# wazzuck/multimodal-image-transformer

Measured on AMD Instinct MI355X. Metric: image-caption pairs/sec (train step), 6L/d512 decoder + ViT-B/16, 1/2/4/8 GPU, higher is better.
Workload: dtype bf16; 1 GPU; configs[1]: 6L d512 decoder + ViT-B/16 (197 patches), batch 64/GPU, seq_len 64; global_batch=64, seq_len=64, vocab=10000, memory_mode=patches, parallelism=dp1

## Files before the change

### include/mit_hip.h

```cpp
#ifndef MIT_HIP_H
#define MIT_HIP_H

#include <stdint.h>

#ifdef __cplusplus
extern "C" {
#endif

#define MIT_OK 0
#define MIT_ERR_INVALID 1
#define MIT_ERR_HIP 2

enum { MIT_F32 = 0, MIT_BF16 = 1 };
enum { MIT_K_CONTIG = 0, MIT_MN_CONTIG = 1 };
enum { MIT_ACT_NONE = 0, MIT_ACT_RELU = 1, MIT_ACT_GELU = 2, MIT_ACT_QUICK_GELU = 3 };
#define MIT_ARGMAX_SLOTS 16
enum { MIT_DECODE_ATTN_BH = 0, MIT_DECODE_ATTN_ROWS = 1, MIT_DECODE_ATTN_ROWS_NT = 2 };

const char* mit_last_error(void);
int mit_abi_version(void);

void* mit_plan_begin(void);
void* mit_plan_end(void);
long mit_plan_size(const void* plan);
// ... 79 lines not shown
  long k_row, k_batch;
  const void* v;
  long v_row, v_batch;
  void* o;
  long o_row, o_batch;
  float* lse;
  const int64_t* key_tokens;
  long tok_batch;
  int pad_idx;
  int causal;
  float scale;
  float drop_p;
  const uint64_t* seed;
  uint32_t site;
} mit_attn_args;
int mit_attention_fwd(int dtype, long B, long H, long Lq, long Lk, long Dh, const mit_attn_args* a, void* stream);

typedef struct {
  const void* dout;
  long do_row, do_batch;
  void* dq;
  long dq_row, dq_batch;
  void* dk;
  long dk_row, dk_batch;
  void* dv;
  long dv_row, dv_batch;
  float* delta_ws;
} mit_attn_grads;
int mit_attention_bwd(int dtype, long B, long H, long Lq, long Lk, long Dh, const mit_attn_args* a,
                      const mit_attn_grads* g, void* stream);

int mit_attention_set_index_limit(double limit);

enum { MIT_ATTN_GENERIC = 0, MIT_ATTN_FWD_MFMA = 1, MIT_ATTN_FWD_HEAD = 2, MIT_ATTN_FWD_HEAD_DROP = 3 };
enum { MIT_ATTN_BWD_MFMA = 1, MIT_ATTN_BWD_HEAD = 2 };
typedef struct {
  int fwd, fwd_nw, fwd_lkp;
  int bwd, bwd_nw, bwd_lkp;
} mit_attn_plan;
int mit_attention_plan(int dtype, long B, long H, long Lq, long Lk, long Dh, const mit_attn_args* a,
                       const mit_attn_grads* g, mit_attn_plan* plan);

int mit_im2col(int dtype, long B, long C, long H, long W, long P, const float* img, void* out, long kpad, void* stream);
int mit_vit_assemble(int dtype, long B, long np, long E, const void* patch, const float* cls, const float* pos, void* h,
                     void* stream);
enum { MIT_ELT_SCALAR = 0, MIT_ELT_VEC8 = 1 };
int mit_im2col_plan(int dtype, long B, long C, long H, long W, long P, const float* img, const void* out, long kpad);
int mit_vit_assemble_plan(int dtype, long B, long np, long E, const void* patch, const float* cls, const float* pos,
                          const void* h);

int mit_embed_fwd(int dtype, long B, long T, long d, const int64_t* tokens, const void* table, float scale,
                  const float* pe, float drop_p, const uint64_t* seed, uint32_t site, void* out, void* stream);
long mit_embed_plan_ints(long n);
int mit_embed_plan(const int64_t* tokens, long n, int* plan, void* stream);
int mit_embed_plan_keys_per_thread(long n);
int mit_embed_bwd(int dtype, long B, long T, long d, const int64_t* tokens, const void* dx, float scale, float drop_p,
                  const uint64_t* seed, uint32_t site, int pad_idx, const int* plan, float* dtable, void* stream);

enum { MIT_CE_BLOCK = 0, MIT_CE_ROWS = 1 };
int mit_cross_entropy_plan(int dtype, long rows, long V, const void* logits, long ld, const float* row_loss);
int mit_count_targets(const int64_t* targets, long n, int ignore_index, float* count, void* stream);
int mit_cross_entropy(int dtype, long rows, long V, void* logits, long ld, const int64_t* targets, int ignore_index,
                      const float* count, float* loss_sum, int want_grad, float* row_loss, void* stream);
int mit_scalar_div(const float* a, const float* b, float* out, void* stream);

int mit_colsum(int dtype, long M, long N, const void* dy, long ld, float* out, int accumulate, float* ws, void* stream);
long mit_colsum_ws_floats(long M, long N);
// ... 157 lines not shown
```

### multimodal-image-transformer_amd/csrc/attention.hip

```cpp
#include "common.h"

namespace {

constexpr int D = 64;

struct AttnK {
  const void* q;
  long q_row, q_batch;
  const void* k;
  long k_row, k_batch;
  const void* v;
  long v_row, v_batch;
  void* o;
  long o_row, o_batch;
  float* lse;
  const int64_t* tok;
  long tok_batch;
  int pad;
  int causal;
  float scale;
  const uint64_t* seed;
  uint32_t site;
  uint32_t thresh;
  float dscale;
// ... 387 lines not shown
#pragma unroll
  for (int i = 0; i < 4; ++i) {
    typedef __attribute__((ext_vector_type(4))) __bf16 bf16x4;
    bf16x4 o4 = {(bf16)(ot[i][0] * inv), (bf16)(ot[i][1] * inv), (bf16)(ot[i][2] * inv), (bf16)(ot[i][3] * inv)};
    *(bf16x4*)(O + i * 16 + g * 4) = o4;
  }
  if (a.lse && g == 0) a.lse[(b * H + h) * Lq + qi] = (m + __log2f(l)) * 0.6931471805599453f;
}

constexpr int HK_MAX = 640;
constexpr int HS = 4;
constexpr int HS_DROP = 8;

__device__ __forceinline__ float xmax_rows(float v) {
  const auto a = __builtin_amdgcn_permlane16_swap(__float_as_uint(v), __float_as_uint(v), false, false);
  v = __builtin_fmaxf(__uint_as_float(a[0]), __uint_as_float(a[1]));
  const auto b = __builtin_amdgcn_permlane32_swap(__float_as_uint(v), __float_as_uint(v), false, false);
  return __builtin_fmaxf(__uint_as_float(b[0]), __uint_as_float(b[1]));
}
__device__ __forceinline__ float xsum_rows(float v) {
  const auto a = __builtin_amdgcn_permlane16_swap(__float_as_uint(v), __float_as_uint(v), false, false);
  v = __uint_as_float(a[0]) + __uint_as_float(a[1]);
  const auto b = __builtin_amdgcn_permlane32_swap(__float_as_uint(v), __float_as_uint(v), false, false);
  return __uint_as_float(b[0]) + __uint_as_float(b[1]);
}
__device__ __forceinline__ float max16(const float (&s)[16]) {
  const float a = __builtin_fmaxf(__builtin_fmaxf(s[0], s[1]), s[2]), b = __builtin_fmaxf(__builtin_fmaxf(s[3], s[4]), s[5]);
  const float c = __builtin_fmaxf(__builtin_fmaxf(s[6], s[7]), s[8]), d = __builtin_fmaxf(__builtin_fmaxf(s[9], s[10]), s[11]);
  const float e = __builtin_fmaxf(__builtin_fmaxf(s[12], s[13]), s[14]);
  return __builtin_fmaxf(__builtin_fmaxf(__builtin_fmaxf(a, b), c), __builtin_fmaxf(__builtin_fmaxf(d, e), s[15]));
}
constexpr bf16x8 ones8 = {(bf16)1.0f, (bf16)1.0f, (bf16)1.0f, (bf16)1.0f, (bf16)1.0f, (bf16)1.0f, (bf16)1.0f, (bf16)1.0f};

template <bool DROP>
__global__ __attribute__((amdgpu_flat_work_group_size(64, DROP ? 512 : 1024))) void attn_fwd_head(long H, long Lq, long Lk, AttnK a, int kbytes, int vbytes,
                                                      int lkp) {
  extern __shared__ __attribute__((aligned(16))) char lds[];
  char* Ks = lds;
  char* Vs = lds + (long)lkp * 128;
  constexpr int HSN = DROP ? HS_DROP : HS;
  const int tid = threadIdx.x, lane = tid & 63, w = tid >> 6, g = lane >> 4, nw = blockDim.x >> 6;
  const long h = blockIdx.x, b = blockIdx.y;
  MIT_DASSERT(h < H && Lk <= lkp && lkp <= HK_MAX && Lq > 0);
  const bf16* Kb = (const bf16*)a.k + b * a.k_batch + h * D;
  const bf16* Vb = (const bf16*)a.v + b * a.v_batch + h * D;
  const __amdgpu_buffer_rsrc_t rk = __builtin_amdgcn_make_buffer_rsrc((void*)Kb, (short)0, kbytes, 0x00020000);
  const __amdgpu_buffer_rsrc_t rv = __builtin_amdgcn_make_buffer_rsrc((void*)Vb, (short)0, vbytes, 0x00020000);
  const int nid = lkp * 8;
  for (int base = tid; base < nid; base += HSN * (int)blockDim.x) {
    u32x4 kv[HSN], vv[HSN];
#pragma unroll
    for (int u = 0; u < HSN; ++u) {
      const int id = base + u * (int)blockDim.x, r = id >> 3, c = id & 7;
      const bool ok = r < Lk;
      kv[u] = __builtin_bit_cast(u32x4, __builtin_amdgcn_raw_buffer_load_b128(
                                            rk, (int)(ok ? (uint32_t)((r * a.k_row + c * 8) * 2) : A_OOB), 0, 0));
      vv[u] = __builtin_bit_cast(u32x4, __builtin_amdgcn_raw_buffer_load_b128(
                                            rv, (int)(ok ? (uint32_t)((r * a.v_row + c * 8) * 2) : A_OOB), 0, 0));
    }
#pragma unroll
    for (int u = 0; u < HSN; ++u) {
      const int id = base + u * (int)blockDim.x, r = id >> 3, c = id & 7;
      if (id < nid) {
        *(u32x4*)(Ks + koff_k(r, c)) = kv[u];
        *(u32x4*)(Vs + koff_v(r, c * 16)) = vv[u];
      }
    }
  }
  __syncthreads();

  const float sl2 = a.scale * 1.4426950408889634f;
  const uint64_t key = DROP ? site_key(a.seed, a.site) : 0ull;
  const int nqt = (int)((Lq + 15) / 16);
  const int q = (lane & 15) >> 2, pp = lane & 3;
  const int kofs = koff_k(lane & 15, g);
  const int kofs1 = koff_k(lane & 15, 4 + g);
  int vofs[4][2];
#pragma unroll
  for (int i = 0; i < 4; ++i) {
    const int colb = (i * 16 + 4 * pp) * 2;
    vofs[i][0] = koff_v(g * 4 + q, colb);
    vofs[i][1] = koff_v(16 + g * 4 + q, colb);
  }
  for (int qt = w; qt < nqt; qt += nw) {
    const long qi = (long)qt * 16 + (lane & 15);
    const bool qlive = qi < Lq;
    bf16x8 qf[2];
    {
      const bf16* Qr = (const bf16*)a.q + b * a.q_batch + h * D + (qlive ? qi : 0) * a.q_row;
#pragma unroll
      for (int kk = 0; kk < 2; ++kk) {
        u32x4 v = *(const u32x4*)(Qr + kk * 32 + g * 8);
        if (!qlive) v = u32x4{0u, 0u, 0u, 0u};
        qf[kk] = __builtin_bit_cast(bf16x8, v);
      }
    }
    const uint32_t rowbase = ((uint32_t)(b * H + h) * (uint32_t)Lq + (uint32_t)qi) * (uint32_t)Lk + (uint32_t)(g * 4);
    const uint32_t kf = key_fold(key);
    f32x4 ot[4];
#pragma unroll
    for (int i = 0; i < 4; ++i) ot[i] = f32x4{0.f, 0.f, 0.f, 0.f};
    float m = -INFINITY, l = 0.f;
    f32x4 lacc = {0.f, 0.f, 0.f, 0.f};
    const char* Kc = Ks;
    const char* Vc = Vs;
    int j0 = 0;
    const int ilk = (int)Lk;
    for (; j0 + 64 <= lkp; j0 += 64, Kc += 64 * 128, Vc += 64 * 128) {
      f32x4 st[4];
#pragma unroll
      for (int nb = 0; nb < 4; ++nb) {
        const u32x4 k0 = *(const u32x4*)(Kc + nb * 2048 + kofs);
        const u32x4 k1 = *(const u32x4*)(Kc + nb * 2048 + kofs1);
        st[nb] = __builtin_amdgcn_mfma_f32_16x16x32_bf16(__builtin_bit_cast(bf16x8, k0), qf[0],
                                                          f32x4{0.f, 0.f, 0.f, 0.f}, 0, 0, 0);
        st[nb] = __builtin_amdgcn_mfma_f32_16x16x32_bf16(__builtin_bit_cast(bf16x8, k1), qf[1], st[nb], 0, 0, 0);
      }
      s16x8 vv[2][4];
#pragma unroll
      for (int hh = 0; hh < 2; ++hh)
#pragma unroll
        for (int i = 0; i < 4; ++i) {
          s16x4 lo = __builtin_amdgcn_ds_read_tr16_b64_v4i16(LDS_PTR(s16x4, Vc + hh * 4096 + vofs[i][0]));
          s16x4 hi = __builtin_amdgcn_ds_read_tr16_b64_v4i16(LDS_PTR(s16x4, Vc + hh * 4096 + vofs[i][1]));
          vv[hh][i] = s16x8{lo[0], lo[1], lo[2], lo[3], hi[0], hi[1], hi[2], hi[3]};
        }
      float s[16];
#pragma unroll
      for (int nb = 0; nb < 4; ++nb)
// ... 92 lines not shown
#pragma unroll
        for (int i = 0; i < 4; ++i) {
          const s16x4 lo = __builtin_amdgcn_ds_read_tr16_b64_v4i16(LDS_PTR(s16x4, Vc + vofs[i][0]));
          const s16x4 hi = __builtin_amdgcn_ds_read_tr16_b64_v4i16(LDS_PTR(s16x4, Vc + vofs[i][1]));
          const s16x8 vv = {lo[0], lo[1], lo[2], lo[3], hi[0], hi[1], hi[2], hi[3]};
          ot[i] = __builtin_amdgcn_mfma_f32_16x16x32_bf16(__builtin_bit_cast(bf16x8, vv), pb, ot[i], 0, 0, 0);
        }
      }
      if (ntail & 1) {
        const int tb = ntail - 1;
        const int voff = tb == 2 ? 4096 : 0;
        typedef __attribute__((ext_vector_type(4))) __bf16 bf16x4;
        bf16x4 pq;
#pragma unroll
        for (int t = 0; t < 4; ++t) pq[t] = (bf16)p[(tb == 2 ? 8 : 0) + t];
#pragma unroll
        for (int i = 0; i < 4; ++i) {
          const s16x4 lo = __builtin_amdgcn_ds_read_tr16_b64_v4i16(LDS_PTR(s16x4, Vc + voff + vofs[i][0]));
          ot[i] = __builtin_amdgcn_mfma_f32_16x16x16bf16_1k(lo, __builtin_bit_cast(s16x4, pq), ot[i], 0, 0, 0);
        }
      }
    }
    if (qlive) {
      const float inv = 1.0f / l;
      bf16* O = (bf16*)a.o + b * a.o_batch + qi * a.o_row + h * D;
#pragma unroll
      for (int i = 0; i < 4; ++i) {
        typedef __attribute__((ext_vector_type(4))) __bf16 bf16x4;
        bf16x4 o4 = {(bf16)(ot[i][0] * inv), (bf16)(ot[i][1] * inv), (bf16)(ot[i][2] * inv), (bf16)(ot[i][3] * inv)};
        *(bf16x4*)(O + i * 16 + g * 4) = o4;
      }
      if (a.lse && g == 0) a.lse[(b * H + h) * Lq + qi] = (m + __log2f(l)) * 0.6931471805599453f;
    }
  }
}

__device__ __forceinline__ bf16x8 lds_row_frag(const char* tile, int row, int chunk) {
  return __builtin_bit_cast(bf16x8, *(const u32x4*)(tile + koff_k(row, chunk)));
}
__device__ __forceinline__ bf16x8 lds_tr_frag(const char* tile, int kbase, int c0, int lane) {
  const int g = lane >> 4, q = (lane & 15) >> 2, p = lane & 3;
  const int colb = (c0 + 4 * p) * 2;
  const int r0 = kbase + g * 4 + q;
  auto addr = [&](int r) { return r * 128 + ((((colb >> 4) ^ ((r >> 1) & 7)) << 4) | (colb & 15)); };
  s16x4 lo = __builtin_amdgcn_ds_read_tr16_b64_v4i16(LDS_PTR(s16x4, tile + addr(r0)));
  s16x4 hi = __builtin_amdgcn_ds_read_tr16_b64_v4i16(LDS_PTR(s16x4, tile + addr(r0 + 16)));
  s16x8 v = {lo[0], lo[1], lo[2], lo[3], hi[0], hi[1], hi[2], hi[3]};
  return __builtin_bit_cast(bf16x8, v);
}
__device__ __forceinline__ void load_tile_rows(char* tile, const bf16* base, long row_stride, long r0, long nrows, int bytes,
                                               int tid) {
  const __amdgpu_buffer_rsrc_t rs = __builtin_amdgcn_make_buffer_rsrc((void*)base, (short)0, bytes, 0x00020000);
#pragma unroll
  for (int i = 0; i < 2; ++i) {
    const int id = tid + 256 * i, r = id >> 3, c = id & 7;
    const long row = r0 + r;
    const uint32_t off = row < nrows ? (uint32_t)((row * row_stride + c * 8) * 2) : A_OOB;
    *(u32x4*)(tile + koff_k(r, c)) = __builtin_bit_cast(u32x4, __builtin_amdgcn_raw_buffer_load_b128(rs, (int)off, 0, 0));
  }
}

struct AttnBwdBytes {
  int q, k, v, dO;
};

__global__ __launch_bounds__(256) void attn_bwd_dq_mfma(long H, long Lq, long Lk, AttnK a, AttnG gr, AttnBwdBytes nb_) {
// ... 373 lines not shown
    switch (dh) {                               \
      case 16: { constexpr int DH = 16; __VA_ARGS__; } break;   \
      case 32: { constexpr int DH = 32; __VA_ARGS__; } break;   \
      case 64: { constexpr int DH = 64; __VA_ARGS__; } break;   \
      default: { constexpr int DH = 128; __VA_ARGS__; } break;  \
    }                                           \
  } while (0)

inline bool head_dim_ok(long dh) { return dh == 16 || dh == 32 || dh == 64 || dh == 128; }

AttnK make_k(const mit_attn_args* x) {
  AttnK a;
  a.q = x->q; a.q_row = x->q_row; a.q_batch = x->q_batch;
  a.k = x->k; a.k_row = x->k_row; a.k_batch = x->k_batch;
  a.v = x->v; a.v_row = x->v_row; a.v_batch = x->v_batch;
  a.o = x->o; a.o_row = x->o_row; a.o_batch = x->o_batch;
  a.lse = x->lse; a.tok = x->key_tokens; a.tok_batch = x->tok_batch; a.pad = x->pad_idx;
  a.causal = x->causal; a.scale = x->scale; a.seed = x->seed; a.site = x->site;
  a.dropout = x->drop_p > 0.f;
  a.thresh = drop_threshold(x->drop_p);
  a.dscale = x->drop_p < 1.f ? 1.f / (1.f - x->drop_p) : 0.f;
  return a;
}

}


static double g_idx32_limit = 4294967296.0;
extern "C" int mit_attention_set_index_limit(double limit) {
  g_idx32_limit = limit > 0 ? limit : 4294967296.0;
  return MIT_OK;
}

constexpr int PLAN_SPAN = -1;
struct FwdPlan {
  int family;
  int nw, lkp;
  long kb, vb;
};
struct BwdPlan {
  int family;
  int lkp;
  AttnBwdBytes nb;
};

static FwdPlan plan_fwd(int dtype, long B, long H, long Lq, long Lk, long Dh, const mit_attn_args* x) {
  FwdPlan p{MIT_ATTN_GENERIC, 0, 0, 0, 0};
  const bool mfma_ok = Dh == D && dtype == MIT_BF16 && x->q_row % 8 == 0 && x->q_batch % 8 == 0 && x->k_row % 8 == 0 &&
                       x->k_batch % 8 == 0 && x->v_row % 8 == 0 && x->v_batch % 8 == 0 && x->o_row % 4 == 0 &&
                       x->o_batch % 4 == 0 && ((uintptr_t)x->q | (uintptr_t)x->k | (uintptr_t)x->v) % 16 == 0 &&
                       ((uintptr_t)x->o % 8) == 0;
  if (!mfma_ok) return p;
  p.kb = 2 * ((Lk - 1) * x->k_row + D);
  p.vb = 2 * ((Lk - 1) * x->v_row + D);
  if (p.kb >= (1L << 31) || p.vb >= (1L << 31)) {
    p.family = PLAN_SPAN;
    return p;
  }
  const bool dropout = x->drop_p > 0.f;
  const bool idx32 = !dropout || (double)B * (double)H * (double)Lq * (double)Lk < g_idx32_limit;
  if (!x->causal && !x->key_tokens && Lk <= HK_MAX && H <= 65535 && B <= 65535 && idx32) {
    constexpr int pad = 16;
    p.lkp = (int)((Lk + pad - 1) / pad * pad);
    const int nqt = (int)((Lq + 15) / 16);
    const int maxw = (dropout || 2 * p.lkp * 256 <= 160 * 1024) ? 8 : 16;
    p.nw = std::min(nqt, maxw);
    p.family = dropout ? MIT_ATTN_FWD_HEAD_DROP : MIT_ATTN_FWD_HEAD;
  } else if (idx32) {
    p.family = MIT_ATTN_FWD_MFMA;
  }
  return p;
}

static BwdPlan plan_bwd(int dtype, long B, long H, long Lq, long Lk, long Dh, const mit_attn_args* x,
                        const mit_attn_grads* gg) {
  BwdPlan p{MIT_ATTN_GENERIC, 0, {0, 0, 0, 0}};
  auto al = [](const void* ptr, int n) { return ((uintptr_t)ptr % n) == 0; };
  const bool mfma_ok = Dh == D && dtype == MIT_BF16 && x->q_row % 8 == 0 && x->q_batch % 8 == 0 && x->k_row % 8 == 0 &&
                       x->k_batch % 8 == 0 && x->v_row % 8 == 0 && x->v_batch % 8 == 0 && x->o_row % 8 == 0 &&
                       x->o_batch % 8 == 0 && gg->do_row % 8 == 0 && gg->do_batch % 8 == 0 && gg->dq_row % 4 == 0 &&
                       gg->dq_batch % 4 == 0 && gg->dk_row % 4 == 0 && gg->dk_batch % 4 == 0 && gg->dv_row % 4 == 0 &&
                       gg->dv_batch % 4 == 0 && al(x->q, 16) && al(x->k, 16) && al(x->v, 16) && al(x->o, 16) &&
                       al(gg->dout, 16) && al(gg->dq, 8) && al(gg->dk, 8) && al(gg->dv, 8);
  if (!mfma_ok) return p;
  const long qb = 2 * ((Lq - 1) * x->q_row + D), kb = 2 * ((Lk - 1) * x->k_row + D);
  const long vb = 2 * ((Lk - 1) * x->v_row + D), db = 2 * ((Lq - 1) * gg->do_row + D);
  if (!(qb < (1L << 31) && kb < (1L << 31) && vb < (1L << 31) && db < (1L << 31))) {
    p.family = PLAN_SPAN;
    return p;
  }
  p.nb.q = (int)qb;
  p.nb.k = (int)kb;
  p.nb.v = (int)vb;
  p.nb.dO = (int)db;
  if (Lq <= 64 && Lk <= HB_MAXK && H <= 65535 && B <= 65535 && x->o_row % 8 == 0 &&
      (double)B * (double)H * (double)Lq * (double)Lk < g_idx32_limit) {
    p.lkp = (int)((Lk + 31) / 32 * 32);
    p.family = MIT_ATTN_BWD_HEAD;
  } else {
    p.family = MIT_ATTN_BWD_MFMA;
  }
  return p;
}

extern "C" int mit_attention_plan(int dtype, long B, long H, long Lq, long Lk, long Dh, const mit_attn_args* x,
                                  const mit_attn_grads* gg, mit_attn_plan* out) {
  MIT_CHECK_ARG(x && out, "mit_attention_plan: null pointer");
  MIT_CHECK_ARG(dtype == MIT_BF16 || dtype == MIT_F32, "mit_attention_plan: bad dtype %d", dtype);
  MIT_CHECK_ARG(head_dim_ok(Dh), "mit_attention_plan: head_dim %ld unsupported (16, 32, 64, 128)", Dh);
  MIT_CHECK_ARG(B > 0 && H > 0 && Lq > 0 && Lk > 0, "mit_attention_plan: empty problem");
  const FwdPlan f = plan_fwd(dtype, B, H, Lq, Lk, Dh, x);
  MIT_CHECK_ARG(f.family != PLAN_SPAN, "mit_attention_plan: K/V span >= 2 GiB");
  const bool head = f.family == MIT_ATTN_FWD_HEAD || f.family == MIT_ATTN_FWD_HEAD_DROP;
  *out = mit_attn_plan{f.family, head ? f.nw : 0, head ? f.lkp : 0, -1, 0, 0};
  if (gg) {
    const BwdPlan b = plan_bwd(dtype, B, H, Lq, Lk, Dh, x, gg);
    MIT_CHECK_ARG(b.family != PLAN_SPAN, "mit_attention_plan: operand span >= 2 GiB");
    out->bwd = b.family;
    out->bwd_nw = b.family == MIT_ATTN_BWD_HEAD ? HB_NT / 64 : 0;
    out->bwd_lkp = b.family == MIT_ATTN_BWD_HEAD ? b.lkp : 0;
  }
  return MIT_OK;
}

extern "C" int mit_attention_fwd(int dtype, long B, long H, long Lq, long Lk, long Dh, const mit_attn_args* x,
                                 void* stream) {
  MIT_CHECK_ARG(x && x->q && x->k && x->v && x->o, "mit_attention_fwd: null pointer");
  MIT_RECORD([=, c = *x]() { return mit_attention_fwd(dtype, B, H, Lq, Lk, Dh, &c, stream); });
  MIT_CHECK_ARG(head_dim_ok(Dh), "mit_attention_fwd: head_dim %ld unsupported (16, 32, 64, 128)", Dh);
  if (B <= 0 || H <= 0 || Lq <= 0) return MIT_OK;
  MIT_CHECK_ARG(Lk > 0, "mit_attention_fwd: Lk must be > 0");
  AttnK a = make_k(x);
  hipStream_t s = (hipStream_t)stream;
  dim3 grid((unsigned)((Lq + 63) / 64), (unsigned)H, (unsigned)B);
  const FwdPlan p = plan_fwd(dtype, B, H, Lq, Lk, Dh, x);
  MIT_CHECK_ARG(p.family != PLAN_SPAN, "mit_attention_fwd: K/V span >= 2 GiB");
  if (p.family == MIT_ATTN_FWD_HEAD || p.family == MIT_ATTN_FWD_HEAD_DROP) {
    const int lds = p.lkp * 256;
    static bool attr = false;
    if (!attr) {
      (void)hipFuncSetAttribute((const void*)attn_fwd_head<false>, hipFuncAttributeMaxDynamicSharedMemorySize,
                                HK_MAX * 256);
      (void)hipFuncSetAttribute((const void*)attn_fwd_head<true>, hipFuncAttributeMaxDynamicSharedMemorySize,
                                HK_MAX * 256);
      attr = true;
    }
    dim3 hg((unsigned)H, (unsigned)B);
    if (p.family == MIT_ATTN_FWD_HEAD_DROP)
      hipLaunchKernelGGL(attn_fwd_head<true>, hg, dim3(64 * p.nw), lds, s, H, Lq, Lk, a, (int)p.kb, (int)p.vb, p.lkp);
    else
      hipLaunchKernelGGL(attn_fwd_head<false>, hg, dim3(64 * p.nw), lds, s, H, Lq, Lk, a, (int)p.kb, (int)p.vb, p.lkp);
  } else if (p.family == MIT_ATTN_FWD_MFMA) {
    hipLaunchKernelGGL(attn_fwd_mfma, grid, dim3(256), 0, s, H, Lq, Lk, a, (int)p.kb, (int)p.vb);
  } else if (dtype == MIT_BF16) {
    DISPATCH_DH(Dh, hipLaunchKernelGGL((attn_fwd_simple<bf16, DH>), grid, dim3(64), 0, s, H, Lq, Lk, a));
  } else {
    DISPATCH_DH(Dh, hipLaunchKernelGGL((attn_fwd_simple<float, DH>), grid, dim3(64), 0, s, H, Lq, Lk, a));
  }
  MIT_LAUNCH_CHECK("mit_attention_fwd");
  return MIT_OK;
}

extern "C" int mit_attention_bwd(int dtype, long B, long H, long Lq, long Lk, long Dh, const mit_attn_args* x,
                                 const mit_attn_grads* gg, void* stream) {
  MIT_CHECK_ARG(x && gg && x->q && x->k && x->v && x->o && x->lse, "mit_attention_bwd: null forward pointer");
  MIT_CHECK_ARG(gg->dout && gg->dq && gg->dk && gg->dv && gg->delta_ws, "mit_attention_bwd: null grad pointer");
  MIT_RECORD([=, c = *x, cg = *gg]() { return mit_attention_bwd(dtype, B, H, Lq, Lk, Dh, &c, &cg, stream); });
  MIT_CHECK_ARG(head_dim_ok(Dh), "mit_attention_bwd: head_dim %ld unsupported (16, 32, 64, 128)", Dh);
  if (B <= 0 || H <= 0 || Lq <= 0 || Lk <= 0) return MIT_OK;
  AttnK a = make_k(x);
// ... 34 lines not shown
```

### multimodal-image-transformer_amd/native.py

```python
from __future__ import annotations

import ctypes
import os
from typing import Optional

os.environ.setdefault("GPU_MAX_HW_QUEUES", "8")

import torch
from torch.utils._python_dispatch import TorchDispatchMode

_HERE = os.path.dirname(os.path.abspath(__file__))
LIB_PATH = os.environ.get("MIT_HIP_LIB", os.path.join(_HERE, "lib", "libmit_hip.so"))
ABI_VERSION = 9
ARGMAX_SLOTS = 16

F32, BF16 = 0, 1
K_CONTIG, MN_CONTIG = 0, 1
ACT_NONE, ACT_RELU, ACT_GELU, ACT_QUICK_GELU = 0, 1, 2, 3


class NativeError(RuntimeError):
    pass


# ... 24 lines not shown
                ("c_row", L), ("c_batch", L), ("kv_col0", L), ("pos", vp), ("argmax_keys", vp)]


class DecodeGemmPlan(ctypes.Structure):
    _fields_ = [("a_mode", I), ("act", I), ("r_mode", I), ("c_f32", I), ("waves", I), ("block_rows", I),
                ("grid", L), ("lds_bytes", L)]


DECODE_ATTN_BH, DECODE_ATTN_ROWS, DECODE_ATTN_ROWS_NT = 0, 1, 2
DECODE_ATTN_FP8_BH, DECODE_ATTN_FP8_ROWS = 3, 4


class LnGradsJob(ctypes.Structure):
    _fields_ = [("rows", L), ("cols", L), ("ws", vp), ("dgamma", vp), ("dbeta", vp)]


class AttnArgs(ctypes.Structure):
    _fields_ = [("q", vp), ("q_row", L), ("q_batch", L), ("k", vp), ("k_row", L), ("k_batch", L),
                ("v", vp), ("v_row", L), ("v_batch", L), ("o", vp), ("o_row", L), ("o_batch", L),
                ("lse", vp), ("key_tokens", vp), ("tok_batch", L), ("pad_idx", I), ("causal", I),
                ("scale", Fl), ("drop_p", Fl), ("seed", vp), ("site", U32)]


class AttnGrads(ctypes.Structure):
    _fields_ = [("dout", vp), ("do_row", L), ("do_batch", L), ("dq", vp), ("dq_row", L), ("dq_batch", L),
                ("dk", vp), ("dk_row", L), ("dk_batch", L), ("dv", vp), ("dv_row", L), ("dv_batch", L),
                ("delta_ws", vp)]


class AttnPlan(ctypes.Structure):
    _fields_ = [("fwd", I), ("fwd_nw", I), ("fwd_lkp", I), ("bwd", I), ("bwd_nw", I), ("bwd_lkp", I)]


ATTN_GENERIC, ATTN_FWD_MFMA, ATTN_FWD_HEAD, ATTN_FWD_HEAD_DROP = 0, 1, 2, 3
ATTN_BWD_MFMA, ATTN_BWD_HEAD = 1, 2


class LnPlan(ctypes.Structure):
    _fields_ = [("fwd", I), ("fwd_nv", I), ("bwd", I), ("bwd_nv", I)]


LN_SCALAR, LN_VEC4, LN_WIDE, LN_PAIR = 0, 1, 2, 3
CE_BLOCK, CE_ROWS = 0, 1
ELT_SCALAR, ELT_VEC8 = 0, 1
SCORE_STREAM, SCORE_REGS = 0, 1


SIGNATURES = {
    "mit_last_error": (ctypes.c_char_p, []),
    "mit_abi_version": (I, []),
    "mit_gemm": (I, [ctypes.POINTER(GemmArgs), vp]),
    "mit_gemm_workspace_bytes": (L, [L, L, L]),
    "mit_gemm_set_variant": (I, [I]),
    "mit_gemm_plan": (I, [ctypes.POINTER(GemmArgs), ctypes.POINTER(I)]),
    "mit_gemm_grouped_ws_bytes": (L, [ctypes.POINTER(GemmArgs), I]),
    "mit_gemm_grouped": (I, [ctypes.POINTER(GemmArgs), I, ctypes.POINTER(LnGradsJob), I, vp, L, vp]),
    "mit_layernorm_fwd": (I, [I, L, L, vp, L, vp, L, Fl, vp, U32, vp, vp, Fl, vp, vp, L, vp, vp, vp]),
    "mit_layernorm_fwd_x32": (I, [L, L, vp, L, vp, L, vp, vp, vp, Fl, vp, I, L, vp]),
    "mit_residual_out": (I, [L, L, vp, L, vp, L, vp, L, vp]),
    "mit_row_stats64": (I, [L, L, vp, L, vp, vp]),
    "mit_layernorm_bwd_ws_floats": (L, [L, L]),
    "mit_layernorm_bwd": (I, [I, L, L, vp, vp, vp, vp, vp, vp, vp, Fl, vp, U32, vp, vp, vp, vp]),
    "mit_layernorm_param_grads": (I, [L, L, vp, vp, vp, vp]),
    "mit_layernorm_plan": (I, [I, L, L, vp, L, vp, L, vp, vp, L, vp, vp, vp, vp, vp, ctypes.POINTER(LnPlan)]),
    "mit_attention_fwd": (I, [I, L, L, L, L, L, ctypes.POINTER(AttnArgs), vp]),
    "mit_attention_bwd": (I, [I, L, L, L, L, L, ctypes.POINTER(AttnArgs), ctypes.POINTER(AttnGrads), vp]),
    "mit_attention_set_index_limit": (I, [ctypes.c_double]),
    "mit_attention_plan": (I, [I, L, L, L, L, L, ctypes.POINTER(AttnArgs), ctypes.POINTER(AttnGrads),
                               ctypes.POINTER(AttnPlan)]),
    "mit_im2col": (I, [I, L, L, L, L, L, vp, vp, L, vp]),
    "mit_vit_assemble": (I, [I, L, L, L, vp, vp, vp, vp, vp]),
    "mit_im2col_plan": (I, [I, L, L, L, L, L, vp, vp, L]),
    "mit_vit_assemble_plan": (I, [I, L, L, L, vp, vp, vp, vp]),
    "mit_cross_entropy_plan": (I, [I, L, L, vp, L, vp]),
    "mit_embed_plan_keys_per_thread": (I, [L]),
    "mit_embed_fwd": (I, [I, L, L, L, vp, vp, Fl, vp, Fl, vp, U32, vp, vp]),
    "mit_embed_bwd": (I, [I, L, L, L, vp, vp, Fl, Fl, vp, U32, I, vp, vp, vp]),
    "mit_embed_plan_ints": (L, [L]),
    "mit_embed_plan": (I, [vp, L, vp, vp]),
    "mit_count_targets": (I, [vp, L, I, vp, vp]),
    "mit_cross_entropy": (I, [I, L, L, vp, L, vp, I, vp, vp, I, vp, vp]),
    "mit_colsum": (I, [I, L, L, vp, L, vp, I, vp, vp]),
    "mit_colsum_ws_floats": (L, [L, L]),
    "mit_grad_norm_ws_floats": (L, [L]),
    "mit_grad_norm": (I, [vp, L, Fl, vp, vp, vp]),
    "mit_step_inc": (I, [vp, vp]),
    "mit_stamp": (I, [vp, I, vp]),
    "mit_adamw": (I, [L, vp, vp, vp, vp, vp, vp, vp, vp, Fl, Fl, Fl, Fl, vp]),
    "mit_grad_accumulate_blocks": (L, [L]),
    "mit_grad_accumulate": (I, [L, vp, vp, I, vp]),
    "mit_cast_f32": (I, [I, L, vp, vp, vp]),
    "mit_zero": (I, [vp, L, vp]),
    "mit_scalar_div": (I, [vp, vp, vp, vp]),
    "mit_dropout_mask": (I, [L, Fl, vp, U32, vp, vp]),
    "mit_attention_decode": (I, [I, L, L, L, vp, L, vp, L, L, vp, L, L, vp, L, L, vp, vp, L, I, Fl, vp]),
    "mit_attention_decode_plan": (I, [I, L, L, L, vp, L, vp, L, L, vp, L, L, vp, L, L, vp, vp]),
    "mit_decode_gemm_plan": (I, [ctypes.POINTER(DecodeGemmArgs), ctypes.POINTER(DecodeGemmPlan)]),
    "mit_kv_store": (I, [I, L, L, vp, L, vp, L, L, vp, vp]),
    "mit_embed_decode": (I, [I, L, L, vp, L, vp, vp, Fl, vp, vp, vp]),
    "mit_image_normalize": (I, [L, L, L, vp, vp, ctypes.POINTER(Fl), ctypes.POINTER(Fl), vp]),
# ... 25 lines not shown
    "mit_attention_decode_fp8": (I, [L, L, L, vp, L, vp, L, L, vp, L, L, vp, vp, L, vp, L, L, L, Fl, vp]),
    "mit_attention_decode_fp8_plan": (I, [L, L, L, vp, L, vp, L, L, vp, L, L, vp, vp, L, vp, L, L, L]),
    "mit_attention_decode_ragged": (I, [I, L, L, L, vp, L, vp, L, L, vp, L, L, vp, L, L, vp, vp, L, I, Fl, vp]),
    "mit_attention_decode_ragged_plan": (I, [I, L, L, L, vp, L, vp, L, L, vp, L, L, vp, L, L, vp, vp]),
    "mit_kv_store_ragged": (I, [I, L, L, vp, L, vp, L, L, vp, vp]),
    "mit_embed_decode_ragged": (I, [I, L, L, vp, L, vp, vp, Fl, vp, vp, vp]),
    "mit_greedy_pick_ragged": (I, [L, L, vp, L, vp, L, vp, ctypes.c_int64, vp, vp, vp, vp]),
    "mit_greedy_pick_keys_ragged": (I, [L, vp, vp, L, vp, ctypes.c_int64, vp, vp, vp, vp]),
    "mit_slot_admit": (I, [L, vp, L, L, L, vp, L, vp, L, vp, vp, L, vp, L, ctypes.c_int64, vp, vp, vp, vp, vp]),
    "mit_logits_constrain_ragged": (I, [L, L, vp, L, vp, L, vp, vp, Fl, L, L, ctypes.c_int64, vp, L, vp, L, L, vp, vp]),
    "mit_sample_pick_ragged": (I, [L, L, vp, L, Fl, L, Fl, vp, vp, vp, vp, L, vp, ctypes.c_int64, vp, vp, vp, vp, vp,
                                   vp]),
    "mit_slot_admit_ex": (I, [L, vp, L, L, L, vp, L, vp, L, vp, vp, L, vp, L, ctypes.c_int64, vp, vp, vp, vp, vp, vp,
                              vp, vp, vp]),
}


def load_library(path: str = None) -> ctypes.CDLL:
    global _lib
    if _lib is not None:
        return _lib
    path = path or os.environ.get("MIT_LIB") or LIB_PATH
    if not os.path.exists(path):
        raise NativeError(f"libmit_hip.so not found at {path}: build it with `python __graft_entry__.py build` "
                          f"(or `make -C multimodal-image-transformer_amd/csrc`). There is no CPU fallback.")
    lib = ctypes.CDLL(path)
    for name, (res, args) in SIGNATURES.items():
        fn = getattr(lib, name)
        fn.restype = res
        fn.argtypes = args
    if lib.mit_abi_version() != ABI_VERSION:
        raise NativeError(f"{path}: ABI version {lib.mit_abi_version()}, this binding needs {ABI_VERSION}: rebuild it")
    _lib = lib
    return lib


def lib() -> ctypes.CDLL:
    return _lib if _lib is not None else load_library()


TORCH_OPS_PATH = os.path.join(_HERE, "lib", "libmit_torch_ops.so")
_torch_ops_loaded = False


def load_torch_ops(path: str = None):
    global _torch_ops_loaded
    if not _torch_ops_loaded:
        p = path or TORCH_OPS_PATH
        if not os.path.exists(p):
            raise NativeError(f"libmit_torch_ops.so not found at {p}: build it with `python __graft_entry__.py build`")
        torch.ops.load_library(p)
        _torch_ops_loaded = True
    return torch.ops.mit_hip


def require_gpu():
    if not torch.cuda.is_available():
        raise NativeError("multimodal-image-transformer_amd kernels need a ROCm GPU (MI355X / gfx950); none is "
                          "visible. The product path has no CPU fallback.")


def _check(rc: int, name: str):
    if rc != 0:
        msg = lib().mit_last_error()
        raise NativeError(f"{name} failed (rc={rc}): {msg.decode() if msg else ''}")

# ... 236 lines not shown
    jobs = (LnGradsJob * max(1, len(ln_jobs)))()
    for i, (rows, cols, lws, dg, db) in enumerate(ln_jobs):
        jobs[i] = LnGradsJob(rows, cols, ptr(lws), ptr(dg), ptr(db))
    wsb = workspace.numel() * workspace.element_size()

    def launch():
        _check(lib().mit_gemm_grouped(arr, len(problems), jobs, len(ln_jobs), ptr(workspace), wsb, stream_ptr()),
               "mit_gemm_grouped")
    probe = _gemm_probe
    if probe is None:
        launch()
        return
    flops = sum(2.0 * M * N * K for _, _, _, M, N, K, _, _, _ in problems)
    nbytes = sum(2 * K * (M + N) + 4 * M * N for _, _, _, M, N, K, _, _, _ in problems)
    probe.grouped(flops, nbytes, launch)


_gemm_probe = None


def gemm_relaunch(g, stream) -> None:
    _check(lib().mit_gemm(ctypes.byref(g), stream), "mit_gemm")


def set_gemm_probe(probe):
    global _gemm_probe
    _gemm_probe = probe


def attention_set_index_limit(limit: float = 0.0):
    _check(lib().mit_attention_set_index_limit(float(limit)), "mit_attention_set_index_limit")


def gemm_set_variant(v):
    _check(lib().mit_gemm_set_variant(int(v)), "mit_gemm_set_variant")


def gemm_plan(g):
    ks = ctypes.c_int(1)
    tile = lib().mit_gemm_plan(ctypes.byref(g), ctypes.byref(ks))
    return tile, ks.value


def gemm_workspace_bytes(M, N, K):
    return lib().mit_gemm_workspace_bytes(M, N, K)


def gemm_workspace(M, N, K, device=None):
    return torch.zeros(max(gemm_workspace_bytes(M, N, K), 4096) // 4 + 4, dtype=torch.float32, device=device)


def linear(x, w, out, *, bias=None, act=ACT_NONE, residual=None, drop_p=0.0, seed=None, site=0, workspace=None,
           tiles=0):
    M, K = x.shape[0], x.shape[-1]
    N = w.shape[0]
    gemm(x, w, out, M, N, K, lda=x.stride(0), bias=bias, act=act, residual=residual, drop_p=drop_p, seed=seed,
         site=site, workspace=workspace, tiles=tiles)


def layernorm_fwd(x, gamma, beta, eps, y, *, r=None, drop_p=0.0, seed=None, site=0, z=None, mean=None, rstd=None,
                  rows=None, cols=None, ldx=None, ldr=None, ldy=None):
    cols = cols if cols is not None else x.shape[-1]
    rows = rows if rows is not None else x.numel() // cols
    _check(lib().mit_layernorm_fwd(dtype_code(x), rows, cols, ptr(x), ldx or cols, ptr(r), ldr or cols, drop_p, ptr(seed),
                                   site, ptr(gamma), ptr(beta), eps, ptr(z), ptr(y), ldy or cols, ptr(mean),
                                   ptr(rstd), stream_ptr()), "mit_layernorm_fwd")
# ... 462 lines not shown
```

Before: 13480 pairs/s.

## Add persistent double-buffered head-streaming attention forward kernel behind opt-in mode

Adds a persistent attention forward kernel in which a grid of about one block per CU loops over (batch, head) pairs. It double-buffers K/V in LDS using buffer_load-to-LDS, so staging the next head overlaps compute on the current one, and it prefetches Q fragments one tile ahead. The existing head kernel is also refactored to prefetch Q during K/V staging and on the next tile. The streaming path defaults to OFF and is enabled only via an env var or API call, so by default only the Q-prefetch change runs.

```diff
diff --git a/include/mit_hip.h b/include/mit_hip.h
--- a/include/mit_hip.h
+++ b/include/mit_hip.h
@@ -135,7 +135,11 @@
 
 int mit_attention_set_index_limit(double limit);
 
-enum { MIT_ATTN_GENERIC = 0, MIT_ATTN_FWD_MFMA = 1, MIT_ATTN_FWD_HEAD = 2, MIT_ATTN_FWD_HEAD_DROP = 3 };
+enum { MIT_ATTN_STREAM_RESET = -1, MIT_ATTN_STREAM_AUTO = 0, MIT_ATTN_STREAM_OFF = 1, MIT_ATTN_STREAM_FORCED = 2 };
+int mit_attention_set_head_stream(int mode, int grid);
+
+enum { MIT_ATTN_GENERIC = 0, MIT_ATTN_FWD_MFMA = 1, MIT_ATTN_FWD_HEAD = 2, MIT_ATTN_FWD_HEAD_DROP = 3,
+       MIT_ATTN_FWD_HEAD_STREAM = 4 };
 enum { MIT_ATTN_BWD_MFMA = 1, MIT_ATTN_BWD_HEAD = 2 };
 typedef struct {
   int fwd, fwd_nw, fwd_lkp;
diff --git a/multimodal-image-transformer_amd/csrc/attention.hip b/multimodal-image-transformer_amd/csrc/attention.hip
--- a/multimodal-image-transformer_amd/csrc/attention.hip
+++ b/multimodal-image-transformer_amd/csrc/attention.hip
@@ -443,6 +443,41 @@
 }
 constexpr bf16x8 ones8 = {(bf16)1.0f, (bf16)1.0f, (bf16)1.0f, (bf16)1.0f, (bf16)1.0f, (bf16)1.0f, (bf16)1.0f, (bf16)1.0f};
 
+struct QFrag {
+  u32x4 v[2];
+};
+__device__ __forceinline__ QFrag q_issue(const AttnK& a, long b, long h, long Lq, int qt, int lane) {
+  const long qi = (long)qt * 16 + (lane & 15);
+  const bf16* Qr = (const bf16*)a.q + b * a.q_batch + h * D + (qi < Lq ? qi : 0) * a.q_row;
+  QFrag f;
+#pragma unroll
+  for (int kk = 0; kk < 2; ++kk) f.v[kk] = *(const u32x4*)(Qr + kk * 32 + (lane >> 4) * 8);
+  return f;
+}
+
+struct SweepOfs {
+  int k0, k1;
+  int v[4][2];
+};
+__device__ __forceinline__ SweepOfs sweep_ofs(int lane) {
+  const int g = lane >> 4, q = (lane & 15) >> 2, pp = lane & 3;
+  SweepOfs s;
+  s.k0 = koff_k(lane & 15, g);
+  s.k1 = koff_k(lane & 15, 4 + g);
+#pragma unroll
+  for (int i = 0; i < 4; ++i) {
+    const int colb = (i * 16 + 4 * pp) * 2;
+    s.v[i][0] = koff_v(g * 4 + q, colb);
+    s.v[i][1] = koff_v(16 + g * 4 + q, colb);
+  }
+  return s;
+}
+
+template <bool DROP>
+__device__ __forceinline__ void head_sweep_tile(const AttnK& a, const char* Ks, const char* Vs, const QFrag& qraw, long b,
+                                                long h, long H, long Lq, long Lk, int lkp, int qt, int lane, float sl2,
+                                                uint64_t key, const SweepOfs& so);
+
 template <bool DROP>
 __global__ __attribute__((amdgpu_flat_work_group_size(64, DROP ? 512 : 1024))) void attn_fwd_head(long H, long Lq, long Lk, AttnK a, int kbytes, int vbytes,
                                                       int lkp) {
@@ -453,11 +488,14 @@
   const int tid = threadIdx.x, lane = tid & 63, w = tid >> 6, g = lane >> 4, nw = blockDim.x >> 6;
   const long h = blockIdx.x, b = blockIdx.y;
   MIT_DASSERT(h < H && Lk <= lkp && lkp <= HK_MAX && Lq > 0);
+  const int nqt = (int)((Lq + 15) / 16);
+  QFrag qn{};
   const bf16* Kb = (const bf16*)a.k + b * a.k_batch + h * D;
   const bf16* Vb = (const bf16*)a.v + b * a.v_batch + h * D;
   const __amdgpu_buffer_rsrc_t rk = __builtin_amdgcn_make_buffer_rsrc((void*)Kb, (short)0, kbytes, 0x00020000);
   const __amdgpu_buffer_rsrc_t rv = __builtin_amdgcn_make_buffer_rsrc((void*)Vb, (short)0, vbytes, 0x00020000);
   const int nid = lkp * 8;
+  if (tid >= nid) qn = q_issue(a, b, h, Lq, w, lane);
   for (int base = tid; base < nid; base += HSN * (int)blockDim.x) {
     u32x4 kv[HSN], vv[HSN];
 #pragma unroll
@@ -469,6 +507,7 @@
       vv[u] = __builtin_bit_cast(u32x4, __builtin_amdgcn_raw_buffer_load_b128(
                                             rv, (int)(ok ? (uint32_t)((r * a.v_row + c * 8) * 2) : A_OOB), 0, 0));
     }
+    if (base == tid) qn = q_issue(a, b, h, Lq, w, lane);
 #pragma unroll
     for (int u = 0; u < HSN; ++u) {
       const int id = base + u * (int)blockDim.x, r = id >> 3, c = id & 7;
@@ -482,30 +521,27 @@
 
   const float sl2 = a.scale * 1.4426950408889634f;
   const uint64_t key = DROP ? site_key(a.seed, a.site) : 0ull;
-  const int nqt = (int)((Lq + 15) / 16);
-  const int q = (lane & 15) >> 2, pp = lane & 3;
-  const int kofs = koff_k(lane & 15, g);
-  const int kofs1 = koff_k(lane & 15, 4 + g);
-  int vofs[4][2];
-#pragma unroll
-  for (int i = 0; i < 4; ++i) {
-    const int colb = (i * 16 + 4 * pp) * 2;
-    vofs[i][0] = koff_v(g * 4 + q, colb);
-    vofs[i][1] = koff_v(16 + g * 4 + q, colb);
-  }
+  const SweepOfs so = sweep_ofs(lane);
   for (int qt = w; qt < nqt; qt += nw) {
+    const QFrag qc = qn;
+    if (qt + nw < nqt) qn = q_issue(a, b, h, Lq, qt + nw, lane);
+    head_sweep_tile<DROP>(a, Ks, Vs, qc, b, h, H, Lq, Lk, lkp, qt, lane, sl2, key, so);
+  }
+}
+
+template <bool DROP>
+__device__ __forceinline__ void head_sweep_tile(const AttnK& a, const char* Ks, const char* Vs, const QFrag& qraw, long b,
+                                                long h, long H, long Lq, long Lk, int lkp, int qt, int lane, float sl2,
+                                                uint64_t key, const SweepOfs& so) {
+  const int g = lane >> 4;
+  const int kofs = so.k0, kofs1 = so.k1;
+  const auto& vofs = so.v;
+  {
     const long qi = (long)qt * 16 + (lane & 15);
     const bool qlive = qi < Lq;
     bf16x8 qf[2];
-    {
-      const bf16* Qr = (const bf16*)a.q + b * a.q_batch + h * D + (qlive ? qi : 0) * a.q_row;
-#pragma unroll
-      for (int kk = 0; kk < 2; ++kk) {
-        u32x4 v = *(const u32x4*)(Qr + kk * 32 + g * 8);
-        if (!qlive) v = u32x4{0u, 0u, 0u, 0u};
-        qf[kk] = __builtin_bit_cast(bf16x8, v);
-      }
-    }
+#pragma unroll
+    for (int kk = 0; kk < 2; ++kk) qf[kk] = __builtin_bit_cast(bf16x8, qlive ? qraw.v[kk] : u32x4{0u, 0u, 0u, 0u});
     const uint32_t rowbase = ((uint32_t)(b * H + h) * (uint32_t)Lq + (uint32_t)qi) * (uint32_t)Lk + (uint32_t)(g * 4);
     const uint32_t kf = key_fold(key);
     f32x4 ot[4];
@@ -664,6 +700,74 @@
       }
       if (a.lse && g == 0) a.lse[(b * H + h) * Lq + qi] = (m + __log2f(l)) * 0.6931471805599453f;
     }
+  }
+}
+
+constexpr int HSTREAM_NW = 16;
+constexpr int HSTREAM_MAX = 320;
+
+__global__ __attribute__((amdgpu_flat_work_group_size(64, 1024))) void attn_fwd_head_stream(int H, long Lq, long Lk, AttnK a, int kbytes, int vbytes,
+                                                                                 int lkp, int nheads) {
+  extern __shared__ __attribute__((aligned(16))) char lds[];
+  constexpr int nw = HSTREAM_NW;
+  const int tid = threadIdx.x, lane = tid & 63;
+  const int w = __builtin_amdgcn_readfirstlane(tid >> 6);
+  const int G = gridDim.x;
+  const int img = lkp * 256;
+  const int half = lkp >> 3;
+  MIT_DASSERT((int)blockIdx.x < nheads && blockDim.x == 64 * nw && Lk <= lkp && lkp <= HSTREAM_MAX && (lkp & 15) == 0 &&
+              Lq > 0);
+  const int nqt = (int)((Lq + 15) / 16);
+  const int ns = nqt < nw ? nw - nqt : nw, sw = nqt < nw ? w - nqt : w;
+  auto stage = [&](int hid, char* dst) {
+    if (sw < 0) return;
+    const long b = hid / H, h = hid % H;
+    const uint64_t kb = (uint64_t)((const bf16*)a.k + b * a.k_batch + h * D);
+    const uint64_t vb = (uint64_t)((const bf16*)a.v + b * a.v_batch + h * D);
+    const u32x4 rk = {(uint32_t)kb, (uint32_t)(kb >> 32) & 0xffffu, (uint32_t)kbytes, 0x00020000u};
+    const u32x4 rv = {(uint32_t)vb, (uint32_t)(vb >> 32) & 0xffffu, (uint32_t)vbytes, 0x00020000u};
+    const uint32_t dst0 = (uint32_t)(uintptr_t)LDS_PTR(char, dst);
+    int ln = lane;
+    asm volatile("" : "+v"(ln));
+    for (int i = sw; i < 2 * half; i += ns) {
+      const bool isv = i >= half;
+      const int r = (isv ? i - half : i) * 8 + (ln >> 3), lc = ln & 7;
+      const int c = lc ^ (isv ? ((r >> 1) & 3) << 1 : (r >> 1) & 7);
+      const long ld = isv ? a.v_row : a.k_row;
+      const uint32_t off = r < Lk ? (uint32_t)((r * ld + c * 8) * 2) : A_OOB;
+      asm volatile("s_mov_b32 m0, %0\n\ts_nop 0\n\tbuffer_load_dwordx4 %1, %2, 0 offen lds"
+                   :
+                   : "s"(dst0 + (uint32_t)i * 1024u), "v"(off), "s"(isv ? rv : rk)
+                   : "memory");
+    }
+  };
+  const float sl2 = a.scale * 1.4426950408889634f;
+  const SweepOfs so = sweep_ofs(lane);
+  int hid = blockIdx.x;
+  QFrag qn{};
+  if (w < nqt) qn = q_issue(a, hid / H, hid % H, Lq, w, lane);
+  stage(hid, lds);
+  asm volatile("s_waitcnt vmcnt(0)" ::: "memory");
+  __syncthreads();
+  for (int cur = 0;; cur ^= 1) {
+    const int nxt = hid + G;
+    const bool more = nxt < nheads;
+    QFrag qc = qn;
+    asm volatile("" : "+v"(qc.v[0]), "+v"(qc.v[1]));
+    if (more) stage(nxt, lds + (cur ^ 1) * img);
+    const char* Ks = lds + cur * img;
+    const char* Vs = Ks + lkp * 128;
+    const long b = hid / H, h = hid % H;
+    for (int qt = w; qt < nqt; qt += nw) {
+      if (qt + nw < nqt) qn = q_issue(a, b, h, Lq, qt + nw, lane);
+      else if (more) qn = q_issue(a, nxt / H, nxt % H, Lq, w, lane);
+      head_sweep_tile<false>(a, Ks, Vs, qc, b, h, H, Lq, Lk, lkp, qt, lane, sl2, 0ull, so);
+      qc = qn;
+    }
+    if (!more) break;
+    asm volatile("s_waitcnt vmcnt(0)" ::: "memory");
+    __syncthreads();
+    hid = nxt;
   }
 }
 
@@ -1103,6 +1207,29 @@
   return MIT_OK;
 }
 
+#ifndef MIT_ATTN_STREAM_DEFAULT
+#define MIT_ATTN_STREAM_DEFAULT MIT_ATTN_STREAM_OFF
+#endif
+static int g_stream_mode = MIT_ATTN_STREAM_DEFAULT;
+static int g_stream_grid = 0;
+static int attn_num_cus() {
+  static int n = 0;
+  if (!n) {
+    int dev = 0;
+    hipDeviceProp_t p;
+    n = (hipGetDevice(&dev) == hipSuccess && hipGetDeviceProperties(&p, dev) == hipSuccess) ? p.multiProcessorCount : 256;
+  }
+  return n;
+}
+extern "C" int mit_attention_set_head_stream(int mode, int grid) {
+  MIT_CHECK_ARG(mode == MIT_ATTN_STREAM_RESET || mode == MIT_ATTN_STREAM_AUTO || mode == MIT_ATTN_STREAM_OFF ||
+                    mode == MIT_ATTN_STREAM_FORCED,
+                "mit_attention_set_head_stream: bad mode %d", mode);
+  g_stream_mode = mode == MIT_ATTN_STREAM_RESET ? MIT_ATTN_STREAM_DEFAULT : mode;
+  g_stream_grid = grid > 0 ? grid : 0;
+  return MIT_OK;
+}
+
 constexpr int PLAN_SPAN = -1;
 struct FwdPlan {
   int family;
@@ -1137,6 +1264,13 @@
     const int maxw = (dropout || 2 * p.lkp * 256 <= 160 * 1024) ? 8 : 16;
     p.nw = std::min(nqt, maxw);
     p.family = dropout ? MIT_ATTN_FWD_HEAD_DROP : MIT_ATTN_FWD_HEAD;
+    const bool can_stream = !dropout && p.lkp <= HSTREAM_MAX && B * H < (1L << 31);
+    if (can_stream && (g_stream_mode == MIT_ATTN_STREAM_FORCED ||
+                       (g_stream_mode == MIT_ATTN_STREAM_AUTO && B * H > 2L * attn_num_cus() && nqt > 8 &&
+                        nqt <= HSTREAM_NW))) {
+      p.family = MIT_ATTN_FWD_HEAD_STREAM;
+      p.nw = HSTREAM_NW;
+    }
   } else if (idx32) {
     p.family = MIT_ATTN_FWD_MFMA;
   }
@@ -1182,7 +1316,8 @@
   MIT_CHECK_ARG(B > 0 && H > 0 && Lq > 0 && Lk > 0, "mit_attention_plan: empty problem");
   const FwdPlan f = plan_fwd(dtype, B, H, Lq, Lk, Dh, x);
   MIT_CHECK_ARG(f.family != PLAN_SPAN, "mit_attention_plan: K/V span >= 2 GiB");
-  const bool head = f.family == MIT_ATTN_FWD_HEAD || f.family == MIT_ATTN_FWD_HEAD_DROP;
+  const bool head = f.family == MIT_ATTN_FWD_HEAD || f.family == MIT_ATTN_FWD_HEAD_DROP ||
+                    f.family == MIT_ATTN_FWD_HEAD_STREAM;
   *out = mit_attn_plan{f.family, head ? f.nw : 0, head ? f.lkp : 0, -1, 0, 0};
   if (gg) {
     const BwdPlan b = plan_bwd(dtype, B, H, Lq, Lk, Dh, x, gg);
@@ -1206,7 +1341,18 @@
   dim3 grid((unsigned)((Lq + 63) / 64), (unsigned)H, (unsigned)B);
   const FwdPlan p = plan_fwd(dtype, B, H, Lq, Lk, Dh, x);
   MIT_CHECK_ARG(p.family != PLAN_SPAN, "mit_attention_fwd: K/V span >= 2 GiB");
-  if (p.family == MIT_ATTN_FWD_HEAD || p.family == MIT_ATTN_FWD_HEAD_DROP) {
+  if (p.family == MIT_ATTN_FWD_HEAD_STREAM) {
+    static bool attr = false;
+    if (!attr) {
+      (void)hipFuncSetAttribute((const void*)attn_fwd_head_stream, hipFuncAttributeMaxDynamicSharedMemorySize,
+                                2 * HSTREAM_MAX * 256);
+      attr = true;
+    }
+    const int nheads = (int)(B * H);
+    const int G = std::min(nheads, g_stream_grid > 0 ? g_stream_grid : attn_num_cus());
+    hipLaunchKernelGGL(attn_fwd_head_stream, dim3((unsigned)G), dim3(64 * p.nw), 2 * p.lkp * 256, s, (int)H, Lq, Lk, a,
+                       (int)p.kb, (int)p.vb, p.lkp, nheads);
+  } else if (p.family == MIT_ATTN_FWD_HEAD || p.family == MIT_ATTN_FWD_HEAD_DROP) {
     const int lds = p.lkp * 256;
     static bool attr = false;
     if (!attr) {
diff --git a/multimodal-image-transformer_amd/native.py b/multimodal-image-transformer_amd/native.py
--- a/multimodal-image-transformer_amd/native.py
+++ b/multimodal-image-transformer_amd/native.py
@@ -80,7 +80,8 @@
     _fields_ = [("fwd", I), ("fwd_nw", I), ("fwd_lkp", I), ("bwd", I), ("bwd_nw", I), ("bwd_lkp", I)]
 
 
-ATTN_GENERIC, ATTN_FWD_MFMA, ATTN_FWD_HEAD, ATTN_FWD_HEAD_DROP = 0, 1, 2, 3
+ATTN_GENERIC, ATTN_FWD_MFMA, ATTN_FWD_HEAD, ATTN_FWD_HEAD_DROP, ATTN_FWD_HEAD_STREAM = 0, 1, 2, 3, 4
+ATTN_STREAM_RESET, ATTN_STREAM_AUTO, ATTN_STREAM_OFF, ATTN_STREAM_FORCED = -1, 0, 1, 2
 ATTN_BWD_MFMA, ATTN_BWD_HEAD = 1, 2
 
 
@@ -114,6 +115,7 @@
     "mit_attention_fwd": (I, [I, L, L, L, L, L, ctypes.POINTER(AttnArgs), vp]),
     "mit_attention_bwd": (I, [I, L, L, L, L, L, ctypes.POINTER(AttnArgs), ctypes.POINTER(AttnGrads), vp]),
     "mit_attention_set_index_limit": (I, [ctypes.c_double]),
+    "mit_attention_set_head_stream": (I, [I, I]),
     "mit_attention_plan": (I, [I, L, L, L, L, L, ctypes.POINTER(AttnArgs), ctypes.POINTER(AttnGrads),
                                ctypes.POINTER(AttnPlan)]),
     "mit_im2col": (I, [I, L, L, L, L, L, vp, vp, L, vp]),
@@ -205,6 +207,10 @@
     if lib.mit_abi_version() != ABI_VERSION:
         raise NativeError(f"{path}: ABI version {lib.mit_abi_version()}, this binding needs {ABI_VERSION}: rebuild it")
     _lib = lib
+    mode = os.environ.get("MIT_ATTN_STREAM")
+    if mode:
+        lib.mit_attention_set_head_stream({"auto": ATTN_STREAM_AUTO, "off": ATTN_STREAM_OFF,
+                                           "forced": ATTN_STREAM_FORCED}[mode], 0)
     return lib
 
 
@@ -507,6 +513,10 @@
     _check(lib().mit_attention_set_index_limit(float(limit)), "mit_attention_set_index_limit")
 
 
+def attention_set_head_stream(mode: int = ATTN_STREAM_RESET, grid: int = 0):
+    _check(lib().mit_attention_set_head_stream(int(mode), int(grid)), "mit_attention_set_head_stream")
+
+
 def gemm_set_variant(v):
     _check(lib().mit_gemm_set_variant(int(v)), "mit_gemm_set_variant")
 
```

Result: no change. 13460 pairs/s (-0.1%).
